# mj-will/aspire

Measured on AMD Instinct MI355X. Metric: particle-steps/sec (N x n_steps), 1M particles d=32; log-evidence err vs ref, higher is better.
Workload: dtype f64

## Files before the change

### aspire_amd/csrc/asmc_flow_dev.h

```cpp
#pragma once
#include "asmc_common.h"

typedef float floatx16 __attribute__((ext_vector_type(16)));


__device__ __forceinline__ float flow_standardise(float x, float loc, float scale, float rcp) {
    const float a = x - loc;
    const float q0 = a * rcp;
    const float r = fmaf(-scale, q0, a);
    return fmaf(r, rcp, q0);
}

typedef float flow_std2 __attribute__((ext_vector_type(2)));
__device__ __forceinline__ flow_std2 flow_standardise2(flow_std2 x, flow_std2 loc, flow_std2 scale, flow_std2 rcp) {
    const flow_std2 a = x - loc;
    const flow_std2 q0 = a * rcp;
    const flow_std2 r = __builtin_elementwise_fma(-scale, q0, a);
    return __builtin_elementwise_fma(r, rcp, q0);
}

template <bool INVERSE>
__device__ __forceinline__ void flow_affine(float& x, float sraw, float t, float& ladj, int form) {
    if (form == 0) {
        const float sv = 2.0f - 4.0f * __builtin_amdgcn_rcpf(__expf(sraw) + 1.0f);
// ... 355 lines not shown
    ladj += lacc.x + lacc.y;
}

typedef unsigned flow_u4 __attribute__((ext_vector_type(4)));

template <bool RELU, bool NOP = true, bool PROP = false>
__device__ __forceinline__ void split2_f16(float x0, float x1, unsigned& hp, unsigned& lp) {
    const float v0 = !RELU ? x0 : PROP ? __builtin_elementwise_maximum(x0, 0.0f) : __int_as_float(max(__float_as_int(x0), 0));
    const float v1 = !RELU ? x1 : PROP ? __builtin_elementwise_maximum(x1, 0.0f) : __int_as_float(max(__float_as_int(x1), 0));
    typedef _Float16 half2v __attribute__((ext_vector_type(2)));
    const half2v h = half2v{(_Float16)v0, (_Float16)v1};
    half2v l;
    if (NOP)
        asm("v_fma_mixlo_f16 %0, %1, -1.0, %2 op_sel_hi:[1,0,0]\n\t"
            "v_fma_mixhi_f16 %0, %1, -1.0, %3 op_sel:[1,0,0] op_sel_hi:[1,0,0]\n\t"
            "s_nop 1"
            : "=&v"(l)
            : "v"(h), "v"(v0), "v"(v1));
    else
        asm("v_fma_mixlo_f16 %0, %1, -1.0, %2 op_sel_hi:[1,0,0]\n\t"
            "v_fma_mixhi_f16 %0, %1, -1.0, %3 op_sel:[1,0,0] op_sel_hi:[1,0,0]"
            : "=&v"(l)
            : "v"(h), "v"(v0), "v"(v1));
    hp = __builtin_bit_cast(unsigned, h);
    lp = __builtin_bit_cast(unsigned, l);
}
template <bool SIGNED>
__device__ __forceinline__ void split4_range(unsigned h0, unsigned h1, unsigned& amax_pk) {
    asm("v_pk_maximum3_f16 %0, %0, %1, %2" : "+v"(amax_pk) : "v"(h0), "v"(h1));
    if (SIGNED) asm("v_pk_maximum3_f16 %0, %0, %1, %2 neg_lo:[0,1,1] neg_hi:[0,1,1]" : "+v"(amax_pk) : "v"(h0), "v"(h1));
}
__device__ __forceinline__ float range_pk_max(unsigned amax_pk) {
    typedef _Float16 half2v __attribute__((ext_vector_type(2)));
    const half2v a = __builtin_bit_cast(half2v, amax_pk);
    const float a0 = (float)a[0], a1 = (float)a[1];
    return (a0 != a0 || a1 != a1) ? __builtin_nanf("") : __builtin_fmaxf(a0, a1);
}

template <int H, int W>
__device__ __forceinline__ void coupling_layer_hs2(const float (&condA)[H / 2], float (&transA)[H / 2], const float (&condB)[H / 2],
                                                   float (&transB)[H / 2], const float* __restrict__ lp, int lane, int hh,
                                                   float& ladjA, float& ladjB, unsigned& amaxA, unsigned& amaxB) {
    using FD = FlowDims<H, W>;
    static_assert(H == 16, "one K16 step over the conditioner inputs");
    constexpr int NB1 = FD::NB1, NB3 = FD::NB3, ST1 = H / 16, ST2 = 2 * NB1, G = ST1 + 2 * ST2;
    const float* b1 = lp;
    const float* b2 = b1 + NB1 * 32;
    const float* b3 = b2 + NB1 * 32;
    const float* a1f = b3 + NB3 * 32;
    const half8* A1 = reinterpret_cast<const half8*>(a1f) + lane;
    const half8* A2 = reinterpret_cast<const half8*>(a1f + W * H) + lane;
    const half8* A3 = reinterpret_cast<const half8*>(a1f + W * H + W * W) + lane;
    floatx16 h1A[NB1], h1B[NB1], h2A[NB1], h2B[NB1], oA[NB3], oB[NB3];
    acc_bias1<NB1>(h1A, b1, hh);
    acc_bias1<NB1>(h1B, b1, hh);
    auto src = [&](const float (&cond)[H / 2], const floatx16 (&h1)[NB1], const floatx16 (&h2)[NB1], int g, int j) -> float {
        if (g < ST1) return cond[8 * g + j];
        const int S = (g - ST1) % ST2;
        return g < ST1 + ST2 ? h1[S / 2][8 * (S % 2) + j] : h2[S / 2][8 * (S % 2) + j];
    };
    unsigned hpA[4], lpA[4], hpB[4], lpB[4];
    auto cvtA = [&](int g, int c) {
        const float e0 = src(condA, h1A, h2A, g, 2 * c), e1 = src(condA, h1A, h2A, g, 2 * c + 1);
        if (c == 3) {
            if (g < ST1) split2_f16<false, true>(e0, e1, hpA[c], lpA[c]);
            else split2_f16<true, true>(e0, e1, hpA[c], lpA[c]);
        } else {
            if (g < ST1) split2_f16<false, false>(e0, e1, hpA[c], lpA[c]);
            else split2_f16<true, false>(e0, e1, hpA[c], lpA[c]);
        }
        if (c & 1) {
            if (g < ST1) split4_range<true>(hpA[c - 1], hpA[c], amaxA);
            else split4_range<false>(hpA[c - 1], hpA[c], amaxA);
        }
    };
    auto cvtB = [&](int g, int c) {
        const float e0 = src(condB, h1B, h2B, g, 2 * c), e1 = src(condB, h1B, h2B, g, 2 * c + 1);
        if (c == 3) {
            if (g < ST1) split2_f16<false, true>(e0, e1, hpB[c], lpB[c]);
            else split2_f16<true, true>(e0, e1, hpB[c], lpB[c]);
        } else {
            if (g < ST1) split2_f16<false, false>(e0, e1, hpB[c], lpB[c]);
            else split2_f16<true, false>(e0, e1, hpB[c], lpB[c]);
        }
        if (c & 1) {
            if (g < ST1) split4_range<true>(hpB[c - 1], hpB[c], amaxB);
            else split4_range<false>(hpB[c - 1], hpB[c], amaxB);
        }
    };
    auto pack = [](const unsigned (&q)[4]) -> half8 { return __builtin_bit_cast(half8, flow_u4{q[0], q[1], q[2], q[3]}); };
    flow_f2 laccA = {0.0f, 0.0f}, laccB = {0.0f, 0.0f};
    auto epi = [&](const floatx16 (&o)[NB3], float (&trans)[H / 2], flow_f2& lacc, int c) {
        const int q = 2 * c;
        flow_affine2<false>(trans[q], trans[q + 1], o[q / 16][q % 16], o[(q + 1) / 16][(q + 1) % 16], o[(H / 2 + q) / 16][(H / 2 + q) % 16],
                            o[(H / 2 + q + 1) / 16][(H / 2 + q + 1) % 16], lacc, 0);
    };
#pragma unroll
    for (int c = 0; c < 4; c++) cvtA(0, c);
    half8 bhA = pack(hpA), blA = pack(lpA), bhB, blB;
    __builtin_amdgcn_sched_barrier(0);
#pragma unroll
    for (int g = 0; g < G; g++) {
        const int layer = g < ST1 ? 0 : g < ST1 + ST2 ? 1 : 2;
        const int S = layer == 0 ? g : (g - ST1) % ST2, ST = layer == 0 ? ST1 : ST2;
        const int NBO = layer == 2 ? NB3 : NB1;
        const half8* Ap = layer == 0 ? A1 : layer == 1 ? A2 : A3;
        half8 ah[NB1 > NB3 ? NB1 : NB3], al[NB1 > NB3 ? NB1 : NB3];
#pragma unroll
        for (int nb = 0; nb < NBO; nb++) {
            ah[nb] = Ap[(size_t)(2 * (nb * ST + S)) * 64];
            al[nb] = Ap[(size_t)(2 * (nb * ST + S) + 1) * 64];
        }
        if (layer == 1 && S == 0) {
            acc_bias1<NB1>(h2A, b2, hh);
            acc_bias1<NB1>(h2B, b2, hh);
        }
        if (layer == 2 && S == 0) {
            acc_bias1<NB3>(oA, b3, hh);
            acc_bias1<NB3>(oB, b3, hh);
        }
        const int NM = 3 * NBO;
#pragma unroll
        for (int m = 0; m < NM; m++) {
            const int k = m / NBO, nb = m % NBO;
            floatx16& acc = layer == 0 ? h1A[nb] : layer == 1 ? h2A[nb] : oA[nb];
            acc = __builtin_amdgcn_mfma_f32_32x32x16_f16(k < 2 ? ah[nb] : al[nb], k == 1 ? blA : bhA, acc, 0, 0, 0);
#pragma unroll
            for (int c = 0; c < 4; c++)
                if (c * NM / 4 == m) cvtB(g, c);
            __builtin_amdgcn_sched_barrier(0);
        }
        bhB = pack(hpB), blB = pack(lpB);
#pragma unroll
        for (int m = 0; m < NM; m++) {
            const int k = m / NBO, nb = m % NBO;
            floatx16& acc = layer == 0 ? h1B[nb] : layer == 1 ? h2B[nb] : oB[nb];
            acc = __builtin_amdgcn_mfma_f32_32x32x16_f16(k < 2 ? ah[nb] : al[nb], k == 1 ? blB : bhB, acc, 0, 0, 0);
#pragma unroll
            for (int c = 0; c < 4; c++)
                if (c * NM / 4 == m) {
                    if (g + 1 < G) cvtA(g + 1, c);
                    else epi(oA, transA, laccA, c);
                }
            __builtin_amdgcn_sched_barrier(0);
        }
        if (g + 1 < G) bhA = pack(hpA), blA = pack(lpA);
    }
#pragma unroll
    for (int c = 0; c < 4; c++) epi(oB, transB, laccB, c);
    ladjA += laccA.x + laccA.y;
    ladjB += laccB.x + laccB.y;
}

template <int H, int W, bool PREFETCH = true, int FORM = -1, bool PROP = false>
__device__ __forceinline__ void coupling_layer_hs1p(const float (&cond)[H / 2], float (&trans)[H / 2], const float* __restrict__ lp,
                                                    int lane, int hh, float& ladj, unsigned& amax, int form = 0) {
    using FD = FlowDims<H, W>;
    constexpr int NB1 = FD::NB1, NB3 = FD::NB3, ST1 = H / 16, ST2 = 2 * NB1, G = ST1 + 2 * ST2;
    constexpr int NBM = NB1 > NB3 ? NB1 : NB3;
    const float* b1 = lp;
    const float* b2 = b1 + NB1 * 32;
    const float* b3 = b2 + NB1 * 32;
    const float* a1f = b3 + NB3 * 32;
    const half8* A1 = reinterpret_cast<const half8*>(a1f) + lane;
    const half8* A2 = reinterpret_cast<const half8*>(a1f + W * H) + lane;
    const half8* A3 = reinterpret_cast<const half8*>(a1f + W * H + W * W) + lane;
#ifndef HS1P_EARLY_BIAS
#define HS1P_EARLY_BIAS 0
#endif
    floatx16 h1[NB1], h2[NB1], o[NB3];
    acc_bias1<NB1>(h1, b1, hh);
    if (HS1P_EARLY_BIAS >= 1) acc_bias1<NB1>(h2, b2, hh);
    auto src = [&](int g, int j) -> float {
        if (g < ST1) return cond[8 * g + j];
        const int S = (g - ST1) % ST2;
        return g < ST1 + ST2 ? h1[S / 2][8 * (S % 2) + j] : h2[S / 2][8 * (S % 2) + j];
    };
    auto first_of_layer = [](int g) { return g == 0 || g == ST1 || g == ST1 + ST2; };
    unsigned hp[4], lq[4];
    auto cvt = [&](int g, int c, bool last) {
        const float e0 = src(g, 2 * c), e1 = src(g, 2 * c + 1);
        if (last) {
            if (g < ST1) split2_f16<false, true, PROP>(e0, e1, hp[c], lq[c]);
            else split2_f16<true, true, PROP>(e0, e1, hp[c], lq[c]);
        } else {
            if (g < ST1) split2_f16<false, false, PROP>(e0, e1, hp[c], lq[c]);
            else split2_f16<true, false, PROP>(e0, e1, hp[c], lq[c]);
        }
        if (!PROP && (c & 1)) {
            if (g < ST1) split4_range<true>(hp[c - 1], hp[c], amax);
            else split4_range<false>(hp[c - 1], hp[c], amax);
        }
    };
    auto pack = [](const unsigned (&q)[4]) -> half8 { return __builtin_bit_cast(half8, flow_u4{q[0], q[1], q[2], q[3]}); };
    auto a_ptr = [&](int g) -> const half8* { return g < ST1 ? A1 : g < ST1 + ST2 ? A2 : A3; };
    auto a_load = [&](int g, half8 (&ah)[NBM], half8 (&al)[NBM]) {
        const int layer = g < ST1 ? 0 : g < ST1 + ST2 ? 1 : 2;
        const int S = layer == 0 ? g : (g - ST1) % ST2, ST = layer == 0 ? ST1 : ST2, NBO = layer == 2 ? NB3 : NB1;
        const half8* Ap = a_ptr(g);
#pragma unroll
        for (int nb = 0; nb < NBO; nb++) {
            ah[nb] = Ap[(size_t)(2 * (nb * ST + S)) * 64];
            al[nb] = Ap[(size_t)(2 * (nb * ST + S) + 1) * 64];
        }
    };
#pragma unroll
    for (int c = 0; c < 4; c++) cvt(0, c, c == 3);
    half8 bh = pack(hp), bl = pack(lq);
    half8 ah[NBM], al[NBM], ahn[NBM], aln[NBM];
    a_load(0, ah, al);
    __builtin_amdgcn_sched_barrier(0);
#pragma unroll
    for (int g = 0; g < G; g++) {
        const int layer = g < ST1 ? 0 : g < ST1 + ST2 ? 1 : 2;
        const int NBO = layer == 2 ? NB3 : NB1, NM = 3 * NBO;
        const bool more = g + 1 < G, overlap = more && !first_of_layer(g + 1);
        if (g == ST1 && HS1P_EARLY_BIAS < 1) acc_bias1<NB1>(h2, b2, hh);
        if (g == (HS1P_EARLY_BIAS >= 2 ? ST1 : ST1 + ST2)) acc_bias1<NB3>(o, b3, hh);
        if (PREFETCH && more) a_load(g + 1, ahn, aln);
#pragma unroll
        for (int m = 0; m < NM; m++) {
            const int k = m / NBO, nb = m % NBO;
            floatx16& acc = layer == 0 ? h1[nb] : layer == 1 ? h2[nb] : o[nb];
            acc = __builtin_amdgcn_mfma_f32_32x32x16_f16(k < 2 ? ah[nb] : al[nb], k == 1 ? bl : bh, acc, 0, 0, 0);
            if (overlap) {
#pragma unroll
                for (int c = 0; c < 4; c++)
                    if (c * NM / 4 == m) cvt(g + 1, c, c == 3);
            }
            __builtin_amdgcn_sched_barrier(0);
        }
        if (more) {
            if (!overlap) {
#pragma unroll
                for (int c = 0; c < 4; c++) cvt(g + 1, c, c == 3);
            }
            bh = pack(hp), bl = pack(lq);
            if (PREFETCH) {
#pragma unroll
                for (int nb = 0; nb < NBM; nb++) ah[nb] = ahn[nb], al[nb] = aln[nb];
            } else {
                a_load(g + 1, ah, al);
            }
            __builtin_amdgcn_sched_barrier(0);
        }
    }
    flow_f2 lacc = {0.0f, 0.0f};
#pragma unroll
    for (int q = 0; q < H / 2; q += 2)
        flow_affine2<false>(trans[q], trans[q + 1], o[q / 16][q % 16], o[(q + 1) / 16][(q + 1) % 16], o[(H / 2 + q) / 16][(H / 2 + q) % 16],
                            o[(H / 2 + q + 1) / 16][(H / 2 + q + 1) % 16], lacc, FORM >= 0 ? FORM : form);
    ladj += lacc.x + lacc.y;
}

template <int H, int W, int THREADS>
__device__ __forceinline__ void flow_stage_hs(float* __restrict__ sp, const float* __restrict__ packed, int n_layers) {
    using FD = FlowDims<H, W>;
    constexpr int L4 = FD::LAYER / 4, B4 = FD::BIAS / 4;
    const int total4 = n_layers * L4;
    for (int i4 = threadIdx.x; i4 < total4; i4 += THREADS) {
        const int in_layer = i4 % L4;
        if (in_layer < B4) {
            reinterpret_cast<float4*>(sp)[i4] = reinterpret_cast<const float4*>(packed)[i4];
            continue;
        }
        const int local = in_layer - B4;
        if ((local / 64) & 1) continue;
        const float4 f0 = reinterpret_cast<const float4*>(packed)[i4], f1 = reinterpret_cast<const float4*>(packed)[i4 + 64];
        const float xv[8] = {f0.x, f0.y, f0.z, f0.w, f1.x, f1.y, f1.z, f1.w};
        half8 hi, lo;
        float wmax = 0.0f;
        split8_f16<false>(xv, hi, lo, wmax);
        reinterpret_cast<half8*>(sp)[i4] = hi;
        reinterpret_cast<half8*>(sp)[i4 + 64] = lo;
    }
}
```

### aspire_amd/csrc/asmc_pcn_fused.hip

```cpp
#include <stdlib.h>

#include "asmc_common.h"
#include <type_traits>
#include "asmc_pcn_dev.h"
#include "asmc_flow_dev.h"

#ifndef FUSED_THREADS
#define FUSED_THREADS 512
#endif

#define FUSED_TL_DOUBLES 1368
#define FUSED_MAX_COMPONENTS 4
#ifndef MV_DEPTH
#define MV_DEPTH 4
#endif
typedef double double2v __attribute__((ext_vector_type(2)));
__host__ __device__ constexpr int mv_group(int bi) {
    int g = 0;
    while ((g + 1) * (g + 2) <= bi) g++;
    return g;
}
template <int I, int N, typename F>
__device__ __forceinline__ void mv_for_each(F& f) {
    if constexpr (I < N) {
        f(std::integral_constant<int, I>{});
        mv_for_each<I + 1, N>(f);
    }
}
#ifndef FUSED_INPLACE
#define FUSED_INPLACE 1
#endif
#ifndef FUSED_MVMFMA
#define FUSED_MVMFMA FUSED_INPLACE
#endif
typedef double fused_d4 __attribute__((ext_vector_type(4)));
__device__ __forceinline__ void fused_swap32(double& x, double& y) {
    const unsigned long long xb = __builtin_bit_cast(unsigned long long, x), yb = __builtin_bit_cast(unsigned long long, y);
    const auto lo = __builtin_amdgcn_permlane32_swap((unsigned)xb, (unsigned)yb, false, false);
    const auto hi = __builtin_amdgcn_permlane32_swap((unsigned)(xb >> 32), (unsigned)(yb >> 32), false, false);
    x = __builtin_bit_cast(double, ((unsigned long long)hi[0] << 32) | lo[0]);
    y = __builtin_bit_cast(double, ((unsigned long long)hi[1] << 32) | lo[1]);
}
__device__ __forceinline__ void fused_swap16(double& x, double& y) {
    const unsigned long long xb = __builtin_bit_cast(unsigned long long, x), yb = __builtin_bit_cast(unsigned long long, y);
    const auto lo = __builtin_amdgcn_permlane16_swap((unsigned)xb, (unsigned)yb, false, false);
    const auto hi = __builtin_amdgcn_permlane16_swap((unsigned)(xb >> 32), (unsigned)(yb >> 32), false, false);
    x = __builtin_bit_cast(double, ((unsigned long long)hi[0] << 32) | lo[0]);
    y = __builtin_bit_cast(double, ((unsigned long long)hi[1] << 32) | lo[1]);
}
__device__ __forceinline__ void fused_transpose4(double& q0, double& q1, double& q2, double& q3) {
    fused_swap32(q0, q2);
    fused_swap32(q1, q3);
    fused_swap16(q0, q1);
    fused_swap16(q2, q3);
}
#ifndef HS1P_PREFETCH
#define HS1P_PREFETCH false
#endif
#ifndef FUSED_PRIO_A
#define FUSED_PRIO_A 2
#define FUSED_PRIO_B 1
#endif
#ifndef MV_CHUNK
#define MV_CHUNK 8
#endif
template <typename T, int W, int NOISE, bool HS, int KIND = ASMC_FLOW_COUPLING, bool MIX = false>
__global__ __launch_bounds__(FUSED_THREADS) void k_pcn_flow_fused(
    int64_t n, double* __restrict__ ll, double* __restrict__ lp, double* __restrict__ lq, const double* __restrict__ ptab,
    PcnScalars p, const double* rho_ptr, uint32_t step, const float* __restrict__ packed, int n_layers,
    const float* __restrict__ loc, const float* __restrict__ scale, float ladj0, float base_const,
    unsigned int* __restrict__ tile_counter, long long* __restrict__ block_counts, PcnAdaptArgs ad, int par_words, int affine) {
    constexpr int D = 32, H = 16, THREADS = FUSED_THREADS;
    constexpr int HF = KIND == ASMC_FLOW_MAF ? 32 : H;
    static_assert(KIND == ASMC_FLOW_COUPLING || HS, "the autoregressive variant runs the split-fp16 layers only");
    using FD = FlowDims<HF, W>;
    extern __shared__ __align__(16) float sp[];
    if (HS) {
        flow_stage_hs<HF, W, THREADS>(sp, packed, n_layers);
    } else {
        const int total4 = n_layers * FD::LAYER / 4;
        for (int base = 0; base < total4; base += THREADS * 8) {
            float4 tmp[8];
#pragma unroll
            for (int q = 0; q < 8; q++) {
                const int i4 = base + q * THREADS + threadIdx.x;
                tmp[q] = i4 < total4 ? reinterpret_cast<const float4*>(packed)[i4] : make_float4(0.f, 0.f, 0.f, 0.f);
            }
#pragma unroll
            for (int q = 0; q < 8; q++) {
                const int i4 = base + q * THREADS + threadIdx.x;
                if (i4 < total4) reinterpret_cast<float4*>(sp)[i4] = tmp[q];
            }
        }
    }
    double* tl = reinterpret_cast<double*>(sp + (size_t)n_layers * FD::LAYER);
    constexpr int T_MU = D * D, T_LLMU = T_MU + D, T_LLPR = T_LLMU + D, T_LPMU = T_LLPR + D, T_LPPR = T_LPMU + D,
                  T_LOGW = T_LPPR + D, T_LOC = T_LOGW + 2;
    static_assert(T_LOC + 3 * D / 2 <= FUSED_TL_DOUBLES, "pCN tables");
    constexpr int M_MU = 12 * 64, M_MIX = M_MU + D, M_LOGW = M_MIX + 2 * FUSED_MAX_COMPONENTS * 2 * D, M_LOC = M_LOGW + 2 * FUSED_MAX_COMPONENTS;
    static_assert(M_LOC + 3 * D / 2 <= FUSED_TL_DOUBLES, "pCN tables (matrix-core variant)");
    constexpr bool MVM = FUSED_MVMFMA && FUSED_INPLACE;
    {
        const double* m0g = ptab + 2 * PTAB_TRI(D) + D;
        const int dr = (p.d_noise > 0 && p.d_noise < D) ? p.d_noise : D;
        const int dhalf = KIND == ASMC_FLOW_MAF ? 16 : dr / 2;
        auto nat = [&](int r) -> int {
            const int c = r < 16 ? (r < dhalf ? r : -1) : (r - 16 + dhalf);
            return (c >= 0 && c < dr) ? c : -1;
        };
        if (MVM) {
            for (int e = threadIdx.x; e < 12 * 64; e += THREADS) {
                const int slot = e >> 6, l = e & 63, mb = slot < 4 ? 0 : 1, sidx = slot < 4 ? slot : slot - 4;
                const int i = l & 15, j = nat(16 * mb + 4 * (i & 3) + (i >> 2)), k = 4 * sidx + (l >> 4);
                tl[e] = (j >= 0 && k <= j) ? ptab[j * (j + 1) / 2 + k] : 0.0;
            }
            for (int e = threadIdx.x; e < D; e += THREADS) {
                const int j = nat(16 * ((e >> 2) & 1) + 4 * (e >> 3) + (e & 3));
                tl[M_MU + e] = j >= 0 ? ptab[2 * PTAB_TRI(D) + j] : 0.0;
                reinterpret_cast<float*>(tl + M_LOC)[e] = j >= 0 ? loc[j] : 0.0f;
                reinterpret_cast<float*>(tl + M_LOC)[D + e] = j >= 0 ? scale[j] : 1.0f;
                reinterpret_cast<float*>(tl + M_LOC)[2 * D + e] = j >= 0 ? 1.0f / scale[j] : 1.0f;
            }
            for (int e = threadIdx.x; e < 2 * FUSED_MAX_COMPONENTS * D; e += THREADS) {
                const int tc = e / D, er = e % D, tt = tc / FUSED_MAX_COMPONENTS, c = tc % FUSED_MAX_COMPONENTS;
                const int j = nat(16 * ((er >> 2) & 1) + 4 * (er >> 3) + (er & 3));
                const bool live = j >= 0 && c < (tt == 0 ? p.c_ll : p.c_lp);
                const double* mg = m0g + (size_t)tt * PTAB_MIX(D);
                tl[M_MIX + tc * 2 * D + er] = live ? mg[ASMC_MAX_COMPONENTS + c * D + j] : 0.0;
                tl[M_MIX + tc * 2 * D + D + er] = live ? mg[ASMC_MAX_COMPONENTS * (1 + D) + c * D + j] : 0.0;
            }
            if (threadIdx.x < 2 * FUSED_MAX_COMPONENTS) {
                const int tt = threadIdx.x / FUSED_MAX_COMPONENTS, c = threadIdx.x % FUSED_MAX_COMPONENTS;
                tl[M_LOGW + threadIdx.x] = c < (tt == 0 ? p.c_ll : p.c_lp) ? m0g[(size_t)tt * PTAB_MIX(D) + c] : -INFINITY;
            }
        } else {
            for (int e = threadIdx.x; e < D * D; e += THREADS) {
                const int j = e / D, k = e - j * D;
                tl[e] = k <= j ? ptab[j * (j + 1) / 2 + k] : 0.0;
            }
            for (int e = threadIdx.x; e < D; e += THREADS) {
                tl[T_MU + e] = ptab[2 * PTAB_TRI(D) + e];
                tl[T_LLMU + e] = m0g[ASMC_MAX_COMPONENTS + e];
                tl[T_LLPR + e] = m0g[ASMC_MAX_COMPONENTS * (1 + D) + e];
                tl[T_LPMU + e] = m0g[PTAB_MIX(D) + ASMC_MAX_COMPONENTS + e];
                tl[T_LPPR + e] = m0g[PTAB_MIX(D) + ASMC_MAX_COMPONENTS * (1 + D) + e];
                reinterpret_cast<float*>(tl + T_LOC)[e] = loc[e];
                reinterpret_cast<float*>(tl + T_LOC)[D + e] = scale[e];
                reinterpret_cast<float*>(tl + T_LOC)[2 * D + e] = 1.0f / scale[e];
            }
        }
        if (!MVM && threadIdx.x == 0) tl[T_LOGW] = m0g[0], tl[T_LOGW + 1] = m0g[PTAB_MIX(D)];
    }
    bm_d2* bmt = reinterpret_cast<bm_d2*>(tl + FUSED_TL_DOUBLES);
    if (NOISE == ASMC_NOISE_F64) bm_tab_stage<THREADS>(bmt, p.bmtab);
    unsigned* const par_bits = reinterpret_cast<unsigned*>(bmt + BM_TAB_N);
    for (int wd = threadIdx.x; wd < par_words; wd += THREADS) {
        const uint4 b0 = reinterpret_cast<const uint4*>(p.tile_par)[2 * wd], b1 = reinterpret_cast<const uint4*>(p.tile_par)[2 * wd + 1];
        const unsigned q[8] = {b0.x, b0.y, b0.z, b0.w, b1.x, b1.y, b1.z, b1.w};
        unsigned bits = 0;
#pragma unroll
        for (int k = 0; k < 8; k++) {
            const unsigned nib = (((q[k] & 0x01010101u) * 0x01020408u) >> 24) & 0xFu;
            bits |= nib << (4 * k);
        }
        par_bits[wd] = bits;
    }
    __syncthreads();
    const int lane = threadIdx.x & 63, wave = threadIdx.x >> 6, hh = lane >> 5;
    const bool first_on_simd = __builtin_amdgcn_readfirstlane(wave) < 4;
#ifdef FUSED_STAGGER
    if (!first_on_simd) {
#pragma unroll 1
        for (int i = 0; i < FUSED_STAGGER; i++) __builtin_amdgcn_s_sleep(127);
    }
#endif
    double rho;
    if (ad.prev_cell) {
        const double rp = ad.rho_hist[ad.t - 1];
        if (ad.adapt <= 1) {
            const long long cp = *ad.prev_cell;
            rho = ad.adapt ? pcn_adapt_rho(rp, cp, ad.n, ad.target, ad.t - 1) : rp;
            if (blockIdx.x == 0 && threadIdx.x == 0) ad.counts_out[ad.t - 1] = cp;
        } else if (ad.t % ad.adapt == 0) {
            double r = rp;
            for (int tp = ad.t - ad.adapt; tp < ad.t; tp++) {
                const long long ct = ad.prev_cell[tp % ad.adapt];
                r = pcn_adapt_rho(r, ct, ad.n, ad.target, tp);
                if (blockIdx.x == 0 && threadIdx.x == 0) ad.counts_out[tp] = ct;
            }
            rho = r;
        } else {
            rho = rp;
        }
    } else {
        rho = *rho_ptr;
    }
    if (ad.cell && blockIdx.x == 0 && threadIdx.x == 0) ad.rho_hist[ad.t] = rho;
    const double a = sqrt(1.0 - rho * rho);
    const int dn = __builtin_amdgcn_readfirstlane((p.d_noise > 0 && p.d_noise < 32) ? p.d_noise : 32);
    const int64_t n_tiles = (n + 63) / 64;
    long long n_acc = 0, n_bad = 0;
#ifdef FUSED_STAMP
    unsigned long long tsum[8] = {0, 0, 0, 0, 0, 0, 0, 0}, tprev = 0;
    int ntile = 0;
#define STAMP(k)                                                  \
    do {                                                          \
        __builtin_amdgcn_sched_barrier(0);                        \
        unsigned long long tn_;                                   \
        asm volatile("s_memtime %0\n\ts_waitcnt lgkmcnt(0)" : "=s"(tn_)::"memory"); \
        tsum[k] += tn_ - tprev;                                   \
        tprev = tn_;                                              \
        __builtin_amdgcn_sched_barrier(0);                        \
    } while (0)
#else
#define STAMP(k)
#endif
    const unsigned long long ysa = (unsigned long long)(uintptr_t)p.ys;
    T* ysu = reinterpret_cast<T*>(((unsigned long long)(unsigned)__builtin_amdgcn_readfirstlane((int)(ysa >> 32)) << 32) |
                                  (unsigned)__builtin_amdgcn_readfirstlane((int)(unsigned)ysa));
    const int half_records = (int)__builtin_amdgcn_readfirstlane((int)(unsigned)((unsigned long long)p.n_pad * D * sizeof(T)));
    T* const ysu1 = ysu + (size_t)__builtin_amdgcn_readfirstlane((int)(unsigned)p.n_pad) * D;
    const unsigned ys_row = (unsigned)__builtin_amdgcn_readfirstlane((int)(unsigned)p.n_pad) * (unsigned)sizeof(T);
    const unsigned ys_lane = (unsigned)lane * (unsigned)sizeof(T);
    unsigned char* __restrict__ const tile_par = p.tile_par;
#ifdef FUSED_STAMP
    asm volatile("s_memtime %0\n\ts_waitcnt lgkmcnt(0)" : "=s"(tprev)::"memory");
#endif
#ifdef FUSED_HALF
// ... 202 lines not shown
                return best == -INFINITY ? -INFINITY : best + log(ssum);
            };
            mix_ll = more_components(0, p.c_ll, qa);
            mix_lp = more_components(1, p.c_lp, qb);
        } else {
#ifdef MV_COMPILER
#pragma unroll
        for (int g = 0; g < D / 4; g++) {
            const int j0 = 4 * g;
            double sr[4] = {0.0, 0.0, 0.0, 0.0};
#pragma unroll
            for (int k = 0; k < j0 + 4; k++) {
#pragma unroll
                for (int r = 0; r < 4; r++)
                    if (k <= j0 + r) sr[r] = fma(Lt[(j0 + r) * D + k], v[k], sr[r]);
                if ((k & (MV_CHUNK - 1)) == MV_CHUNK - 1 || k == j0 + 3) asm volatile("" : "+v"(sr[0]), "+v"(sr[1]), "+v"(sr[2]), "+v"(sr[3])::"memory");
            }
#pragma unroll
            for (int r = 0; r < 4; r++) {
                const int j = j0 + r;
                const double xj = (double)(T)(Lt[T_MU + j] + sr[r]);
                const double ta = xj - Lt[T_LLMU + j], tb = xj - Lt[T_LPMU + j];
                qa = fma(ta * ta, Lt[T_LLPR + j], qa);
                qb = fma(tb * tb, Lt[T_LPPR + j], qb);
                xf[j] = flow_standardise((float)xj, locs[j], locs[D + j], locs[2 * D + j]);
            }
            asm volatile("" : "+v"(qa), "+v"(qb), "+v"(xf[j0]), "+v"(xf[j0 + 1]), "+v"(xf[j0 + 2]), "+v"(xf[j0 + 3])::"memory");
        }
#else
        {
            constexpr int NB = (D / 4) * (D / 4 + 1), P = MV_DEPTH;
            const unsigned lbase = (unsigned)(size_t)tl + (unsigned)zoff;
            double2v ring[P][4];
            double sr[4] = {0.0, 0.0, 0.0, 0.0};
            auto issue = [&](auto bc) {
                constexpr int bi = decltype(bc)::value, g = mv_group(bi), b = bi - g * (g + 1), slot = bi % P;
                constexpr int o0 = ((4 * g + 0) * D + 2 * b) * 8, o1 = o0 + D * 8, o2 = o1 + D * 8, o3 = o2 + D * 8;
                auto& rg = ring[slot];
                const unsigned lb = lbase;
                asm volatile("ds_read_b128 %0, %4 offset:%5\n\tds_read_b128 %1, %4 offset:%6\n\t"
                             "ds_read_b128 %2, %4 offset:%7\n\tds_read_b128 %3, %4 offset:%8"
                             : "=&v"(rg[0]), "=&v"(rg[1]), "=&v"(rg[2]), "=&v"(rg[3])
                             : "v"(lb), "n"(o0), "n"(o1), "n"(o2), "n"(o3));
            };
            auto consume = [&](auto bc) {
                constexpr int bi = decltype(bc)::value, g = mv_group(bi), b = bi - g * (g + 1), slot = bi % P, j0 = 4 * g;
                constexpr int ahead = (NB - 1 - bi) < (P - 1) ? (NB - 1 - bi) : (P - 1);
                if constexpr (bi + P - 1 < NB) issue(std::integral_constant<int, (bi + P - 1 < NB ? bi + P - 1 : 0)>{});
                auto& rg = ring[slot];
                static_assert(ahead <= 3, "lgkmcnt holds 15");
                if constexpr (ahead == 0)
                    asm volatile("s_waitcnt lgkmcnt(0)" : "+v"(rg[0]), "+v"(rg[1]), "+v"(rg[2]), "+v"(rg[3]));
                else if constexpr (ahead == 1)
                    asm volatile("s_waitcnt lgkmcnt(4)" : "+v"(rg[0]), "+v"(rg[1]), "+v"(rg[2]), "+v"(rg[3]));
                else if constexpr (ahead == 2)
                    asm volatile("s_waitcnt lgkmcnt(8)" : "+v"(rg[0]), "+v"(rg[1]), "+v"(rg[2]), "+v"(rg[3]));
                else
                    asm volatile("s_waitcnt lgkmcnt(12)" : "+v"(rg[0]), "+v"(rg[1]), "+v"(rg[2]), "+v"(rg[3]));
#pragma unroll
                for (int e = 0; e < 2; e++)
#pragma unroll
                    for (int r = 0; r < 4; r++)
                        if (2 * b + e <= j0 + r) sr[r] = fma(rg[r][e], v[2 * b + e], sr[r]);
                if constexpr (b == 2 * g + 1) {
#pragma unroll
                    for (int r = 0; r < 4; r++) {
                        const int j = j0 + r;
                        const double xj = (double)(T)(Lt[T_MU + j] + sr[r]);
                        const double ta = xj - Lt[T_LLMU + j], tb = xj - Lt[T_LPMU + j];
                        qa = fma(ta * ta, Lt[T_LLPR + j], qa);
                        qb = fma(tb * tb, Lt[T_LPPR + j], qb);
                        xf[j] = flow_standardise((float)xj, locs[j], locs[D + j], locs[2 * D + j]);
                        sr[r] = 0.0;
                    }
                    auto &a0 = qa, &a1 = qb;
                    auto &f0 = xf[j0], &f1 = xf[j0 + 1], &f2 = xf[j0 + 2], &f3 = xf[j0 + 3];
                    asm volatile("" : "+v"(a0), "+v"(a1), "+v"(f0), "+v"(f1), "+v"(f2), "+v"(f3)::"memory");
                }
            };
            mv_for_each<0, (P - 1 < NB ? P - 1 : NB)>(issue);
            mv_for_each<0, NB>(consume);
        }
#endif
        }
        const double nll = MVM ? mix_ll : Lt[T_LOGW] - 0.5 * qa;
        const double nlp = MVM ? mix_lp : Lt[T_LOGW + 1] - 0.5 * qb;
        STAMP(3);
#if !FUSED_INPLACE
        if (valid) {
#pragma unroll
            for (int j = 0; j < D; j++) soa_store<T>(ypr, ys_lane, ys_tile + (unsigned)j * ys_row, v[j]);
        }
#endif
        double t2 = p.beta * (nll + nlp);
        t2 = (t2 < INFINITY) ? t2 : __builtin_nan("");
        double c1 = ref_corr(q1, p.nu, dn);
        double rhs = log_p_t(oll, olp, olq, p.beta) + ref_corr(q0, p.nu, dn);
        double logu = bm_log_unit(accept_uniform(p.seed, gid, step));
        double kll = nll, klp = nlp;
        double kacc = ((t2 + c1) - rhs) - logu;
        asm volatile("" : "+v"(kacc), "+v"(kll), "+v"(klp));
#ifndef FUSED_NOSB
        __builtin_amdgcn_sched_barrier(0);
#endif
        float lqt[2];
        unsigned tn_l = 0;
        float xaA[1][H / 2], xbA[1][H / 2], xaB[1][H / 2], xbB[1][H / 2];
        if constexpr (MVM) {
#pragma unroll
            for (int mb = 0; mb < 2; mb++)
#pragma unroll
                for (int r = 0; r < 4; r++) {
                    const auto sA = __builtin_amdgcn_permlane16_swap(__float_as_uint(xf[(4 * mb + 0) * 4 + r]), __float_as_uint(xf[(4 * mb + 1) * 4 + r]), false, false);
                    const auto sB = __builtin_amdgcn_permlane16_swap(__float_as_uint(xf[(4 * mb + 2) * 4 + r]), __float_as_uint(xf[(4 * mb + 3) * 4 + r]), false, false);
                    if (mb == 0) {
                        xaA[0][r] = __uint_as_float(sA[0]), xaA[0][4 + r] = __uint_as_float(sA[1]);
                        xaB[0][r] = __uint_as_float(sB[0]), xaB[0][4 + r] = __uint_as_float(sB[1]);
                    } else {
                        xbA[0][r] = __uint_as_float(sA[0]), xbA[0][4 + r] = __uint_as_float(sA[1]);
                        xbB[0][r] = __uint_as_float(sB[0]), xbB[0][4 + r] = __uint_as_float(sB[1]);
                    }
                }
        } else {
#pragma unroll
        for (int r = 0; r < H / 2; r++) {
            const auto s1 = __builtin_amdgcn_permlane32_swap(__float_as_uint(xf[r]), __float_as_uint(xf[H / 2 + r]), false, false);
            xaA[0][r] = __uint_as_float(s1[0]);
            xaB[0][r] = __uint_as_float(s1[1]);
            const auto s2 = __builtin_amdgcn_permlane32_swap(__float_as_uint(xf[H + r]), __float_as_uint(xf[H + H / 2 + r]), false, false);
            xbA[0][r] = __uint_as_float(s2[0]);
            xbB[0][r] = __uint_as_float(s2[1]);
        }
        }
        if constexpr (KIND == ASMC_FLOW_MAF) {
            float xA[16], xB[16];
#pragma unroll
            for (int r = 0; r < 8; r++) xA[r] = xaA[0][r], xA[8 + r] = xbA[0][r], xB[r] = xaB[0][r], xB[8 + r] = xbB[0][r];
#ifndef FUSED_NOPRIO
            if (first_on_simd)
                __builtin_amdgcn_s_setprio(FUSED_PRIO_A);
            else
                __builtin_amdgcn_s_setprio(FUSED_PRIO_B);
#endif
            STAMP(4);
            tn_l = tile_fetch();
            auto maf_tile = [&](float(&xv)[16], auto form_c) __attribute__((always_inline)) -> float {
                constexpr int FORM = decltype(form_c)::value;
                float ladj = 0.0f;
                unsigned amax_pk = 0u;
                for (int c = 0; c < n_layers; c++) {
                    float cond[16];
#pragma unroll
                    for (int r = 0; r < 16; r++) cond[r] = xv[r];
                    coupling_layer_hs1p<HF, W, false, FORM, true>(cond, xv, sp + (size_t)c * FD::LAYER, lane, hh, ladj, amax_pk, FORM);
                    __builtin_amdgcn_sched_barrier(0);
                }
                float amax = range_pk_max(amax_pk);
                float q = 0.0f;
#pragma unroll
                for (int r = 0; r < 16; r++) q += xv[r] * xv[r];
                q += __shfl_xor(q, 32);
                const float lj = ladj + __shfl_xor(ladj, 32);
                amax = fmaxf(amax, __shfl_xor(amax, 32));
                return !(amax < FLOW_HS_MAX) ? __builtin_nanf("") : (-0.5f * q + base_const) + (ladj0 + lj);
            };
            if (affine == 0) {
                lqt[0] = maf_tile(xA, std::integral_constant<int, 0>{});
                __builtin_amdgcn_sched_barrier(0);
                STAMP(5);
                lqt[1] = maf_tile(xB, std::integral_constant<int, 0>{});
            } else {
                lqt[0] = maf_tile(xA, std::integral_constant<int, 1>{});
                __builtin_amdgcn_sched_barrier(0);
                STAMP(5);
                lqt[1] = maf_tile(xB, std::integral_constant<int, 1>{});
            }
        } else {
        auto flow_tile = [&](float(&xa)[1][H / 2], float(&xb)[1][H / 2]) __attribute__((always_inline)) -> float {
            float ladj[1] = {0.0f};
            float amax = 0.0f;
#ifndef FUSED_NOFLOW
            for (int c = 0; c < n_layers; c++) {
                const float* lpk = sp + (size_t)c * FD::LAYER;
                if (HS) {
                    if ((c & 1) == 0)
                        coupling_layer_hs<H, W, false, -1, false>(xa[0], xb[0], lpk, lane, hh, ladj[0], amax);
                    else
                        coupling_layer_hs<H, W, false, -1, false>(xb[0], xa[0], lpk, lane, hh, ladj[0], amax);
                } else if ((c & 1) == 0)
                    coupling_layer<H, W, 1>(xa, xb, lpk, lane, hh, ladj);
                else
                    coupling_layer<H, W, 1>(xb, xa, lpk, lane, hh, ladj);
            }
#endif
            float q = 0.0f;
#pragma unroll
            for (int r = 0; r < H / 2; r++) q += xa[0][r] * xa[0][r] + xb[0][r] * xb[0][r];
            q += __shfl_xor(q, 32);
            const float lj = ladj[0] + __shfl_xor(ladj[0], 32);
            amax = fmaxf(amax, __shfl_xor(amax, 32));
            return !(amax < FLOW_HS_MAX) ? __builtin_nanf("") : (-0.5f * q + base_const) + (ladj0 + lj);
        };
#ifndef FUSED_NOPRIO
        if (first_on_simd)
            __builtin_amdgcn_s_setprio(FUSED_PRIO_A);
        else
            __builtin_amdgcn_s_setprio(FUSED_PRIO_B);
#endif
        STAMP(4);
        tn_l = tile_fetch();
#ifndef FUSED_FLOW2
#define FUSED_FLOW2 1
#endif
        if (HS && FUSED_INPLACE) {
            auto one_tile = [&](float(&xa)[1][H / 2], float(&xb)[1][H / 2]) __attribute__((always_inline)) -> float {
                float ladj = 0.0f;
                unsigned amax_pk = 0u;
                for (int c = 0; c < n_layers; c++) {
                    const float* lpk = sp + (size_t)c * FD::LAYER;
                    if ((c & 1) == 0)
                        coupling_layer_hs1p<H, W, HS1P_PREFETCH, 0, true>(xa[0], xb[0], lpk, lane, hh, ladj, amax_pk);
                    else
                        coupling_layer_hs1p<H, W, HS1P_PREFETCH, 0, true>(xb[0], xa[0], lpk, lane, hh, ladj, amax_pk);
                    __builtin_amdgcn_sched_barrier(0);
                }
                float amax = range_pk_max(amax_pk);
                float q = 0.0f;
#pragma unroll
                for (int r = 0; r < H / 2; r++) q += xa[0][r] * xa[0][r] + xb[0][r] * xb[0][r];
                q += __shfl_xor(q, 32);
                const float lj = ladj + __shfl_xor(ladj, 32);
                amax = fmaxf(amax, __shfl_xor(amax, 32));
                return !(amax < FLOW_HS_MAX) ? __builtin_nanf("") : (-0.5f * q + base_const) + (ladj0 + lj);
            };
            lqt[0] = one_tile(xaA, xbA);
            __builtin_amdgcn_sched_barrier(0);
            STAMP(5);
            lqt[1] = one_tile(xaB, xbB);
        } else if (HS && FUSED_FLOW2 && W < 128) {
            float ladjA = 0.0f, ladjB = 0.0f;
            unsigned amaxA = 0u, amaxB = 0u;
            for (int c = 0; c < n_layers; c++) {
                const float* lpk = sp + (size_t)c * FD::LAYER;
                if ((c & 1) == 0)
                    coupling_layer_hs2<H, W>(xaA[0], xbA[0], xaB[0], xbB[0], lpk, lane, hh, ladjA, ladjB, amaxA, amaxB);
                else
                    coupling_layer_hs2<H, W>(xbA[0], xaA[0], xbB[0], xaB[0], lpk, lane, hh, ladjA, ladjB, amaxA, amaxB);
                __builtin_amdgcn_sched_barrier(0);
            }
            auto finish = [&](const float(&xa)[1][H / 2], const float(&xb)[1][H / 2], float ladj, unsigned amax_pk) -> float {
                float amax = range_pk_max(amax_pk);
                float q = 0.0f;
#pragma unroll
                for (int r = 0; r < H / 2; r++) q += xa[0][r] * xa[0][r] + xb[0][r] * xb[0][r];
                q += __shfl_xor(q, 32);
                const float lj = ladj + __shfl_xor(ladj, 32);
                amax = fmaxf(amax, __shfl_xor(amax, 32));
                return !(amax < FLOW_HS_MAX) ? __builtin_nanf("") : (-0.5f * q + base_const) + (ladj0 + lj);
            };
            lqt[0] = finish(xaA, xbA, ladjA, amaxA);
            lqt[1] = finish(xaB, xbB, ladjB, amaxB);
        } else {
            lqt[0] = flow_tile(xaA, xbA);
            __builtin_amdgcn_sched_barrier(0);
            STAMP(5);
            lqt[1] = flow_tile(xaB, xbB);
        }
        }
        __builtin_amdgcn_sched_barrier(0);
        __builtin_amdgcn_s_setprio(0);
        STAMP(6);
        const double nlq = (double)(hh == 0 ? lqt[0] : lqt[1]);
        const bool lq_finite = fabs(nlq) < INFINITY;
        if (valid && !lq_finite) n_bad++;
        const bool accepted = valid && lq_finite && fma(1.0 - p.beta, nlq, kacc) > 0.0;
#if FUSED_INPLACE
        if (accepted) {
            ll[i] = kll;
            lp[i] = klp;
            lq[i] = nlq;
            n_acc++;
        }
        if constexpr (MVM) {
            const unsigned long long accmask = __ballot(accepted);
            const unsigned ys_lane_t = (unsigned)(lane >> 4) * ys_row + (unsigned)(lane & 15) * (unsigned)sizeof(T);
            const __amdgpu_buffer_rsrc_t ysw = __builtin_amdgcn_make_buffer_rsrc(ysu, 0, half_records, 0x00020000);
#pragma unroll
            for (int r = 0; r < 4; r++) {
                if ((accmask >> (16 * r + (lane & 15))) & 1ull) {
#pragma unroll
                    for (int sI = 0; sI < D / 4; sI++)
                        soa_store<T>(ysw, ys_lane_t, ys_tile + (unsigned)(4 * sI) * ys_row + (unsigned)(16 * r) * (unsigned)sizeof(T), v[4 * sI + r]);
                }
            }
        } else if (accepted) {
            const __amdgpu_buffer_rsrc_t ysw = __builtin_amdgcn_make_buffer_rsrc(ysu, 0, half_records, 0x00020000);
#pragma unroll
            for (int j = 0; j < D; j++) soa_store<T>(ysw, ys_lane, ys_tile + (unsigned)j * ys_row, v[j]);
        }
        const unsigned tn = (unsigned)__builtin_amdgcn_readfirstlane((int)tn_l);
        const bool have_n = (int64_t)tn < n_tiles;
        unsigned par_n = 0;
        double vn[D];
#pragma unroll
        for (int j = 0; j < D; j++) vn[j] = 0.0;
        double olln = 0.0, olpn = 0.0, olqn = 0.0;
        if (have_n) {
            par_n = tile_parity(tn);
            tile_load(tn, par_n, vn, olln, olpn, olqn);
        }
#else
        const unsigned tn = (unsigned)__builtin_amdgcn_readfirstlane((int)tn_l);
        const bool have_n = (int64_t)tn < n_tiles;
        unsigned par_n = 0;
        double vn[D];
#pragma unroll
        for (int j = 0; j < D; j++) vn[j] = 0.0;
        double olln = 0.0, olpn = 0.0, olqn = 0.0;
        if (have_n) {
            par_n = tile_parity(tn);
            tile_load(tn, par_n, vn, olln, olpn, olqn);
        }
        if (accepted) {
            ll[i] = kll;
            lp[i] = klp;
            lq[i] = nlq;
            n_acc++;
        }
        {
            const int n_a = __builtin_popcountll(__ballot(accepted)), n_r = __builtin_popcountll(__ballot(valid && !accepted));
            const bool flip = n_a > 0 && n_r <= n_a;
            if (flip ? n_r > 0 : n_a > 0) {
                const __amdgpu_buffer_rsrc_t src = __builtin_amdgcn_make_buffer_rsrc(flip == (par != 0) ? ysu1 : ysu, 0, half_records, 0x00020000);
                const __amdgpu_buffer_rsrc_t dst = __builtin_amdgcn_make_buffer_rsrc(flip == (par != 0) ? ysu : ysu1, 0, half_records, 0x00020000);
                if (valid && accepted != flip) {
                    double w[D];
#pragma unroll
                    for (int j = 0; j < D; j++) w[j] = soa_load<T>(src, ys_lane, ys_tile + (unsigned)j * ys_row);
#pragma unroll
                    for (int j = 0; j < D; j++) soa_store<T>(dst, ys_lane, ys_tile + (unsigned)j * ys_row, w[j]);
                }
            }
            if (flip && lane == 0) tile_par[t] = (unsigned char)(par ^ 1u);
        }
#endif
        STAMP(7);
#ifdef FUSED_STAMP
        ntile++;
#endif
#ifndef FUSED_NOSB
        __builtin_amdgcn_sched_barrier(0);
#endif
        t = tn, par = par_n, have = have_n;
        oll = olln, olp = olpn, olq = olqn;
#pragma unroll
        for (int j = 0; j < D; j++) v[j] = vn[j];
    }
#ifdef FUSED_STAMP
    if (lane == 0 && blockIdx.x == 7 && (wave == 0 || wave == 4) && ntile > 0)
        printf("wave %d tiles %d | fetch %llu yload %llu noise %llu matvec %llu park+swap %llu flowA %llu flowB %llu accept %llu (cycles per tile)\n", wave, ntile,
               tsum[0] / ntile, tsum[1] / ntile, tsum[2] / ntile, tsum[3] / ntile, tsum[4] / ntile, tsum[5] / ntile, tsum[6] / ntile, tsum[7] / ntile);
#endif
    __shared__ long long s_cnt[THREADS / 64];
    n_acc = wave_sum_ll(n_acc);
    n_bad = wave_sum_ll(n_bad);
    if (lane == 0 && n_bad != 0 && ad.nonfinite) atomicAdd(ad.nonfinite, (unsigned long long)n_bad);
    if (lane == 0) s_cnt[wave] = n_acc;
    __syncthreads();
    if (threadIdx.x == 0) {
        long long tsum = 0;
        for (int w = 0; w < THREADS / 64; w++) tsum += s_cnt[w];
        block_counts[blockIdx.x] = tsum;
    }
    if (ad.done == nullptr) return;
    __shared__ int s_last;
    if (threadIdx.x == 0) {
// ... 135 lines not shown
```

Baseline: 3.329 billion.

## Software-pipeline split-fp16 coupling layer with double-buffered weight loads and seam overlap

Restructures the single-tile split-fp16 coupling layer so weight fragments are double-buffered: the high half of the next step's weights is loaded ahead of the current step and the low half just in time. At layer boundaries (seams) it reorders the MFMA loop per output block, moves the bias init one step earlier, and interleaves the next layer's fp16 conversion into the last MFMAs. This aims to hide LDS latency and conversion stalls between layers. It is enabled only for coupling flows with W<=64 and no MIX; otherwise the old plain path is kept. The cost is higher register pressure from the two weight buffers, which may lower occupancy.

```diff
diff --git a/aspire_amd/csrc/asmc_flow_dev.h b/aspire_amd/csrc/asmc_flow_dev.h
--- a/aspire_amd/csrc/asmc_flow_dev.h
+++ b/aspire_amd/csrc/asmc_flow_dev.h
@@ -531,12 +531,14 @@
     ladjB += laccB.x + laccB.y;
 }
 
-template <int H, int W, bool PREFETCH = true, int FORM = -1, bool PROP = false>
+
+template <int H, int W, int FORM = -1, bool PROP = false, int PF_FROM = 1, bool SEAM = true>
 __device__ __forceinline__ void coupling_layer_hs1p(const float (&cond)[H / 2], float (&trans)[H / 2], const float* __restrict__ lp,
                                                     int lane, int hh, float& ladj, unsigned& amax, int form = 0) {
     using FD = FlowDims<H, W>;
     constexpr int NB1 = FD::NB1, NB3 = FD::NB3, ST1 = H / 16, ST2 = 2 * NB1, G = ST1 + 2 * ST2;
     constexpr int NBM = NB1 > NB3 ? NB1 : NB3;
+    constexpr bool SEAMS = SEAM && NB1 >= 2;
     const float* b1 = lp;
     const float* b2 = b1 + NB1 * 32;
     const float* b3 = b2 + NB1 * 32;
@@ -544,12 +546,7 @@
     const half8* A1 = reinterpret_cast<const half8*>(a1f) + lane;
     const half8* A2 = reinterpret_cast<const half8*>(a1f + W * H) + lane;
     const half8* A3 = reinterpret_cast<const half8*>(a1f + W * H + W * W) + lane;
-#ifndef HS1P_EARLY_BIAS
-#define HS1P_EARLY_BIAS 0
-#endif
     floatx16 h1[NB1], h2[NB1], o[NB3];
-    acc_bias1<NB1>(h1, b1, hh);
-    if (HS1P_EARLY_BIAS >= 1) acc_bias1<NB1>(h2, b2, hh);
     auto src = [&](int g, int j) -> float {
         if (g < ST1) return cond[8 * g + j];
         const int S = (g - ST1) % ST2;
@@ -572,55 +569,64 @@
         }
     };
     auto pack = [](const unsigned (&q)[4]) -> half8 { return __builtin_bit_cast(half8, flow_u4{q[0], q[1], q[2], q[3]}); };
-    auto a_ptr = [&](int g) -> const half8* { return g < ST1 ? A1 : g < ST1 + ST2 ? A2 : A3; };
-    auto a_load = [&](int g, half8 (&ah)[NBM], half8 (&al)[NBM]) {
+    auto a_load = [&](int g, half8 (&ah)[NBM], half8 (&al)[NBM], bool hi, bool lo) {
         const int layer = g < ST1 ? 0 : g < ST1 + ST2 ? 1 : 2;
         const int S = layer == 0 ? g : (g - ST1) % ST2, ST = layer == 0 ? ST1 : ST2, NBO = layer == 2 ? NB3 : NB1;
-        const half8* Ap = a_ptr(g);
+        const half8* Ap = layer == 0 ? A1 : layer == 1 ? A2 : A3;
 #pragma unroll
         for (int nb = 0; nb < NBO; nb++) {
-            ah[nb] = Ap[(size_t)(2 * (nb * ST + S)) * 64];
-            al[nb] = Ap[(size_t)(2 * (nb * ST + S) + 1) * 64];
+            if (hi) ah[nb] = Ap[(size_t)(2 * (nb * ST + S)) * 64];
+            if (lo) al[nb] = Ap[(size_t)(2 * (nb * ST + S) + 1) * 64];
         }
     };
+    auto prefetched = [](int g) { return g > 0 && g >= PF_FROM; };
+    half8 ah[2][NBM], al[2][NBM];
+    constexpr bool PLAIN = !SEAMS && PF_FROM >= G;
+    acc_bias1<NB1>(h1, b1, hh);
+    if (!PLAIN) {
+        a_load(0, ah[0], al[0], true, true);
+        __builtin_amdgcn_sched_barrier(0);
+    }
 #pragma unroll
     for (int c = 0; c < 4; c++) cvt(0, c, c == 3);
     half8 bh = pack(hp), bl = pack(lq);
-    half8 ah[NBM], al[NBM], ahn[NBM], aln[NBM];
-    a_load(0, ah, al);
+    if (PLAIN) a_load(0, ah[0], al[0], true, true);
     __builtin_amdgcn_sched_barrier(0);
 #pragma unroll
     for (int g = 0; g < G; g++) {
         const int layer = g < ST1 ? 0 : g < ST1 + ST2 ? 1 : 2;
         const int NBO = layer == 2 ? NB3 : NB1, NM = 3 * NBO;
         const bool more = g + 1 < G, overlap = more && !first_of_layer(g + 1);
-        if (g == ST1 && HS1P_EARLY_BIAS < 1) acc_bias1<NB1>(h2, b2, hh);
-        if (g == (HS1P_EARLY_BIAS >= 2 ? ST1 : ST1 + ST2)) acc_bias1<NB3>(o, b3, hh);
-        if (PREFETCH && more) a_load(g + 1, ahn, aln);
+        const bool seam = SEAMS && more && !overlap;
+        if (g == (SEAMS ? ST1 - 1 : ST1)) acc_bias1<NB1>(h2, b2, hh);
+        if (g == (SEAMS ? ST1 + ST2 - 1 : ST1 + ST2)) acc_bias1<NB3>(o, b3, hh);
+        if (more && prefetched(g + 1)) a_load(g + 1, ah[(g + 1) & 1], al[(g + 1) & 1], true, false);
+        if (prefetched(g)) a_load(g, ah[g & 1], al[g & 1], false, true);
+        if (!PLAIN) __builtin_amdgcn_sched_barrier(0);
 #pragma unroll
         for (int m = 0; m < NM; m++) {
-            const int k = m / NBO, nb = m % NBO;
+            const int k = seam ? m % 3 : m / NBO, nb = seam ? m / 3 : m % NBO;
             floatx16& acc = layer == 0 ? h1[nb] : layer == 1 ? h2[nb] : o[nb];
-            acc = __builtin_amdgcn_mfma_f32_32x32x16_f16(k < 2 ? ah[nb] : al[nb], k == 1 ? bl : bh, acc, 0, 0, 0);
+            acc = __builtin_amdgcn_mfma_f32_32x32x16_f16(k < 2 ? ah[g & 1][nb] : al[g & 1][nb], k == 1 ? bl : bh, acc, 0, 0, 0);
             if (overlap) {
 #pragma unroll
                 for (int c = 0; c < 4; c++)
                     if (c * NM / 4 == m) cvt(g + 1, c, c == 3);
             }
+            if (seam) {
+#pragma unroll
+                for (int c = 0; c < 4; c++)
+                    if (NM - 3 + (c < 2 ? c : 2) == m) cvt(g + 1, c, c == 3);
+            }
             __builtin_amdgcn_sched_barrier(0);
         }
         if (more) {
-            if (!overlap) {
+            if (!overlap && !seam) {
 #pragma unroll
                 for (int c = 0; c < 4; c++) cvt(g + 1, c, c == 3);
             }
             bh = pack(hp), bl = pack(lq);
-            if (PREFETCH) {
-#pragma unroll
-                for (int nb = 0; nb < NBM; nb++) ah[nb] = ahn[nb], al[nb] = aln[nb];
-            } else {
-                a_load(g + 1, ah, al);
-            }
+            if (!prefetched(g + 1)) a_load(g + 1, ah[(g + 1) & 1], al[(g + 1) & 1], true, true);
             __builtin_amdgcn_sched_barrier(0);
         }
     }
diff --git a/aspire_amd/csrc/asmc_pcn_fused.hip b/aspire_amd/csrc/asmc_pcn_fused.hip
--- a/aspire_amd/csrc/asmc_pcn_fused.hip
+++ b/aspire_amd/csrc/asmc_pcn_fused.hip
@@ -54,9 +54,6 @@
     fused_swap16(q0, q1);
     fused_swap16(q2, q3);
 }
-#ifndef HS1P_PREFETCH
-#define HS1P_PREFETCH false
-#endif
 #ifndef FUSED_PRIO_A
 #define FUSED_PRIO_A 2
 #define FUSED_PRIO_B 1
@@ -74,6 +71,8 @@
     constexpr int HF = KIND == ASMC_FLOW_MAF ? 32 : H;
     static_assert(KIND == ASMC_FLOW_COUPLING || HS, "the autoregressive variant runs the split-fp16 layers only");
     using FD = FlowDims<HF, W>;
+    constexpr bool HS1P_SCHED = KIND == ASMC_FLOW_COUPLING && W <= 64 && !MIX;
+    constexpr int HS1P_PF = HS1P_SCHED ? 1 : 1 << 20;
     extern __shared__ __align__(16) float sp[];
     if (HS) {
         flow_stage_hs<HF, W, THREADS>(sp, packed, n_layers);
@@ -582,7 +581,7 @@
                     float cond[16];
 #pragma unroll
                     for (int r = 0; r < 16; r++) cond[r] = xv[r];
-                    coupling_layer_hs1p<HF, W, false, FORM, true>(cond, xv, sp + (size_t)c * FD::LAYER, lane, hh, ladj, amax_pk, FORM);
+                    coupling_layer_hs1p<HF, W, FORM, true, HS1P_PF, HS1P_SCHED>(cond, xv, sp + (size_t)c * FD::LAYER, lane, hh, ladj, amax_pk, FORM);
                     __builtin_amdgcn_sched_barrier(0);
                 }
                 float amax = range_pk_max(amax_pk);
@@ -649,9 +648,9 @@
                 for (int c = 0; c < n_layers; c++) {
                     const float* lpk = sp + (size_t)c * FD::LAYER;
                     if ((c & 1) == 0)
-                        coupling_layer_hs1p<H, W, HS1P_PREFETCH, 0, true>(xa[0], xb[0], lpk, lane, hh, ladj, amax_pk);
+                        coupling_layer_hs1p<H, W, 0, true, HS1P_PF, HS1P_SCHED>(xa[0], xb[0], lpk, lane, hh, ladj, amax_pk);
                     else
-                        coupling_layer_hs1p<H, W, HS1P_PREFETCH, 0, true>(xb[0], xa[0], lpk, lane, hh, ladj, amax_pk);
+                        coupling_layer_hs1p<H, W, 0, true, HS1P_PF, HS1P_SCHED>(xb[0], xa[0], lpk, lane, hh, ladj, amax_pk);
                     __builtin_amdgcn_sched_barrier(0);
                 }
                 float amax = range_pk_max(amax_pk);
```

After: 3.273 billion. 0.983x the previous value.
